# hyllios/CGAT

Hardware: AMD Instinct MI355X
Metric: edges/sec through one CGAT attention layer (fwd+bwd), 1M-edge batch (higher is better)
Workload: dtype f32 storage / f16x3c (24-bit operands: exact h + l + t split, 3 fp16 + 3 six-bit matrix passes where built, six bf16 passes elsewhere; fp32 accumulate); 1 GPU; one GATConvNodes layer (H_Net update) fwd+bwd, 4167 crystals x 20 atoms x 12 nbrs per rank: N=83340, E=1000080, C=Ce=128, H=3, scalar attention; edges_per_rank=1000080, parallelism=dp1 (graphs sharded, gradient all-reduce)

## Files before the change

cgat_amd/csrc/edgebwd.hip:

```cpp
#include <string.h>
#include "../../include/cgat_hip.h"
#include "common.h"
#include "kernels.h"
#include "mfma_bf16.h"

__device__ __forceinline__ float rc_d(unsigned m, int bit) {
  const unsigned s = (unsigned)((int)(m << (31 - bit)) >> 31);
  return __uint_as_float((s & 0x3F800000u) | (~s & 0x3C23D70Au));
}
__device__ __forceinline__ bf16x8 bits8_bf16(unsigned m) {
  uint4 w;
#define GE_BITPAIR(i_) ((((unsigned)((int)(m << (31 - 2 * (i_))) >> 31)) & 0x3F80u) |                     \
                        (((unsigned)((int)(m << (30 - 2 * (i_))) >> 31)) & 0x3F800000u))
  w.x = GE_BITPAIR(0); w.y = GE_BITPAIR(1); w.z = GE_BITPAIR(2); w.w = GE_BITPAIR(3);
#undef GE_BITPAIR
  return __builtin_bit_cast(bf16x8, w);
}
template <int PASSES, bool RC = false, bool BP = false>
__global__ __launch_bounds__(512, 2) void edge_ge_kernel(const float* __restrict__ gZ, long ldg, long gzb,
                                                         const uint4* __restrict__ Wq, int ncb,
                                                         float* __restrict__ out, long ldo,
                                                         const int* __restrict__ scatter, int E, int accumulate,
                                                         const float* __restrict__ bias,
                                                         const float* __restrict__ amax, const EdgeRC rc, HeadBatch hb) {
// ... 996 lines not shown
    {
      CGAT_PROF("edge_gw", stream);
      edge_gw_go(f, p, true, stream);
      CGAT_LAUNCH_CHECK();
    }
    hipLaunchKernelGGL(edge_gw_bit_reduce_kernel, dim3(p.W2 * 4), dim3(256), 0, stream, p.ws + f.slab, f.SM, p.ws + f.slabA, f.SA,
                       p.ws + f.csl, p.rc->wA, p.rc->H, p.rc->HHd, p.W2, f.te_only ? nullptr : p.out, p.ldo, p.te ? *p.te : GwTe{});
    CGAT_LAUNCH_CHECK();
    if (p.te) {
      hipLaunchKernelGGL(gw_te_add_kernel, dim3(cdiv(p.rc->HHd, 256)), dim3(256), 0, stream, p.te->part, p.rc->HHd, p.te->out);
      CGAT_LAUNCH_CHECK();
    }
    if (!f.te_only) return CGAT_OK;
  }
  {
    CGAT_PROF(p.perm ? "edge_gw" : "rows_gw", stream);
    edge_gw_go(f, p, false, stream);
    CGAT_LAUNCH_CHECK();
  }
  return splitk_reduce_launch(p.ws + f.slab, f.S, p.W2, 128, p.out, p.ldo, stream);
}

#define GJ_NODES 4
__global__ __launch_bounds__(256) void edge_gj_kernel(const EdgeRC rc, const int* __restrict__ src_rowptr,
                                                      const int* __restrict__ src_pos, int N, int W2,
                                                      float* __restrict__ Gj, long ldo, float* __restrict__ gjmax) {
  float gmax = 0.f;
  const int per_xcd = gridDim.x / 8;
  const int blk = (blockIdx.x & 7) * per_xcd + (blockIdx.x >> 3);
  const int n0 = blk * GJ_NODES, n1 = min(N, n0 + GJ_NODES);
  for (int q = threadIdx.x; 4 * q < W2; q += 256) {
    const int col = 4 * q;
    const bool isA = col < rc.HHd;
    const int cc = isA ? col : col - rc.HHd, h = cc / rc.Hd;
    const int word = col >> 5, bit = col & 31;
    const float* coef = (isA ? rc.ga : rc.alpha) + h;
    for (int n = n0; n < n1; ++n) {
      const int r0 = src_rowptr[n], r1 = src_rowptr[n + 1];
      float4 acc = make_float4(0.f, 0.f, 0.f, 0.f);
      for (int rb = r0; rb < r1; rb += 4) {
        long t[4];
        float k[4];
        unsigned m[4];
        float4 v[4];
#pragma unroll
        for (int u = 0; u < 4; ++u) t[u] = src_pos[rb + u < r1 ? rb + u : r1 - 1];
#pragma unroll
        for (int u = 0; u < 4; ++u) {
          k[u] = rb + u < r1 ? coef[t[u] * rc.H] : 0.f;
          m[u] = rc.mask[t[u] * rc.nw + word];
          v[u] = *reinterpret_cast<const float4*>(isA ? rc.wA + cc : rc.gS + (long)rc.dst[t[u]] * rc.HHd + cc);
        }
#pragma unroll
        for (int u = 0; u < 4; ++u) {
          const unsigned mb = m[u] >> bit;
          acc.x += (k[u] * v[u].x) * rc_d(mb, 0); acc.y += (k[u] * v[u].y) * rc_d(mb, 1);
          acc.z += (k[u] * v[u].z) * rc_d(mb, 2); acc.w += (k[u] * v[u].w) * rc_d(mb, 3);
        }
      }
      *reinterpret_cast<float4*>(Gj + (long)n * ldo + col) = acc;
      gmax = fmaxf(fmaxf(gmax, fmaxf(fabsf(acc.x), fabsf(acc.y))), fmaxf(fabsf(acc.z), fabsf(acc.w)));
    }
  }
  if (gjmax) block_absmax_commit(gmax, gjmax);
}
int edge_gj_launch(const EdgeRC& rc, const int* src_rowptr, const int* src_pos, int N, int W2, float* Gj, long ldo,
                   hipStream_t stream, float* gjmax) {
  if (N <= 0) return CGAT_OK;
  CGAT_CHECK_ARG(W2 % 4 == 0 && (ldo % 4) == 0 && (((uintptr_t)Gj) & 15) == 0,
                 "edge_gj: W2 = %d must be a multiple of 4 with a 16-byte aligned output", W2);
  CGAT_PROF("edge_gj", stream);
  hipLaunchKernelGGL(edge_gj_kernel, dim3(cdiv(cdiv(N, GJ_NODES), 8) * 8), dim3(256), 0, stream, rc, src_rowptr, src_pos,
                     N, W2, Gj, ldo, gjmax);
  CGAT_LAUNCH_CHECK();
  return CGAT_OK;
}

extern "C" int cgat_debug_edge_bwd_form(int32_t product, int32_t launch, int32_t rows, int32_t W2, int32_t H, int32_t Hd,
                                        int32_t rebuilt, int32_t maxima, int32_t perm, int32_t force_six, int32_t te,
                                        cgat_edge_bwd_form* out) {
  CGAT_CHECK_ARG(out && (product == 0 || product == 1) && launch >= 0 && launch <= (product == 0 ? 3 : 0) && rows >= 0 &&
                 W2 > 0 && W2 % 128 == 0 && H > 0 && Hd > 0, "debug_edge_bwd_form: bad arguments");
  alignas(16) static float present_f;
  static int present_i;
  const EdgeRC rc = edge_rc_shape_only(H, Hd, W2);
  memset(out, 0, sizeof(*out));
  if (product == 1) {
    const EdgeGwParams p = edge_gw_shape(rows, W2, rebuilt ? &rc : nullptr, maxima != 0, perm != 0, force_six != 0, te != 0);
    const EdgeGwForm f = edge_gw_form(p);
    CGAT_TRY(edge_gw_check(p, f));
    out->passes = f.passes; out->rc = f.rc; out->bitplane = f.bitplane; out->grid_x = f.grid_x;
    out->bit_shape = f.bit_shape; out->te_only = f.te_only; out->ranges = f.S; out->SA = f.SA; out->SM = f.SM;
    out->message_pairs = f.npm; out->bit_grid_x = f.bit_grid_x;
    out->ws_end = (int64_t)f.ws_end; out->ws_floats = (int64_t)edge_gw_ws_floats(rows, W2);
    return CGAT_OK;
  }
// ... 14 lines not shown
```

cgat_amd/csrc/kernels.h:

```cpp
#pragma once
#include "common.h"

#define CGAT_ACT_NONE 0
#define CGAT_ACT_TANH 1
#define CGAT_ACT_LEAKY 2
#define CGAT_ACT_RELU 3

struct GemmParams {
  int M, N, K;
  const float* A;
  long lda;
  int a_kmajor;
  const int* a_rgather;
  long a_block;
  const float* B;
  long ldb;
  int b_kmajor;
  const int* b_kgather;
  float* C;
  long ldc;
  const int* c_scatter;
  float alpha, beta;
  const float* bias;
  const float* add1;
// ... 248 lines not shown
  float* out;
  long ld_dact, ld_resid, ld_out;
  int act;
  int dact_type;
  int accumulate;
};
struct ChainDesc {
  ChainLayer layer[CHAIN_MAX];
  int n_layers, rows;
  const float* x;
  long ldx;
  const float* in_dact;
  long ld_in_dact;
  int in_dact_type;
  float* in_store;
  long ld_in_store;
};
int prepare_W_batch_launch(const WPrepBatch& b, float* dst, hipStream_t stream);
bool mlp_chain128_fast(const ChainDesc& d);
int mlp_chain128_launch(const ChainDesc& d, hipStream_t stream);
#define CHAIN_BATCH_MAX 4
int mlp_chain128_batch_launch(const ChainDesc* d, int n, hipStream_t stream);
int edge_seg_bwd_chunks(int N);
int edge_seg_bwd_launch(const float* Z, float* gZ, long gz_block, const float* alpha, const float* gS, const float* gs,
                        const int* rowptr, const float* wA_out, int N, int H, int Hd, float* tt, float* ga, float* Gi,
                        float* partialW, float* gzmax, unsigned* mask, float* gimax, bool vec, bool zb_6, bool zb,
                        bool rc_shape, bool have_scales, hipStream_t stream,
                        const int* bits_src = nullptr);
int attn_signs_launch(const float* Z, const int* perm, long E, int W2, uint8_t* mask, hipStream_t stream,
                      const unsigned* zbits = nullptr);
struct EdgeRC {
  const unsigned* mask;
  const float* ga;
  const float* alpha;
  const float* gS;
  const float* wA;
  const int* dst;
  int H, Hd, HHd, nw;
  const float* cs;
};
bool edge_mma_bf16();
static inline bool edge_rc_shape(int Ce, int H, int Hd) { return Ce == 128 && H > 0 && Hd > 0 && Hd % 128 == 0; }
struct GwTe {
  const float* We;
  long ldw;
  double* part;
  float* out;
};
struct EdgeGeParams {
  const float* gZ;
  long ldg, gzb;
// ... 67 lines not shown
  p.gZ = gZ; p.ldg = ldg; p.gzb = gzb; p.e = e; p.lde = lde; p.perm = perm; p.E = E; p.W2 = W2; p.ws = ws;
  p.out = out; p.ldo = ldo;
  return p;
}
struct EdgeGwForm {
  int passes;
  bool rc;
  bool bit_shape;
  bool bitplane;
  bool te_only;
  int S, grid_x;
  int SA, SM, npm;
  int bit_grid_x;
  size_t slab;
  size_t slabA, csl;
  size_t ws_end;
};
EdgeGwForm edge_gw_form(const EdgeGwParams& p);
bool edge_gw_bitplane_layer(int H, int Hd);
bool edge_gw_dims(int Ce, int W2, long ldg, long gzb);
size_t edge_gw_ws_floats(int E, int W2);
bool edge_gw_force_six(bool on);
int edge_gw_launch(const EdgeGwParams& p, hipStream_t stream);
int edge_gj_launch(const EdgeRC& rc, const int* src_rowptr, const int* src_pos, int N, int W2, float* Gj, long ldo,
                   hipStream_t stream, float* gjmax = nullptr);

bool rows_dw128_fast(const float* G, long ldg, const float* X1, long ldx1, const float* X2, long ldx2);
size_t rows_dw128_ws_bytes(int rows, int nx);
int rows_dw128_launch(const float* G, long ldg, const float* X1, long ldx1, float* out1, long ldo1, const float* X2,
                      long ldx2, float* out2, long ldo2, float* bsum, int rows, void* ws, size_t ws_bytes,
                      hipStream_t stream);
#define DW_BATCH_MAX 32
struct DwBatchItem {
  const float* G;
  const float* X;
  float* out;
  float* bsum;
};
struct DwBatchDesc {
  int n, rows, splits, rows_per_unit;
  long ldg, ldx, ldo;
  DwBatchItem it[DW_BATCH_MAX];
};
size_t rows_dw128_batch_ws_bytes(int n_items, int rows);
bool rows_dw128_batch_fast(const DwBatchDesc& d);
int rows_dw128_batch_launch(DwBatchDesc d, void* ws, size_t ws_bytes, hipStream_t stream);

int layernorm_tanh_fwd_launch(const float* u, float* y, int rows, int W, float eps, hipStream_t s);
// ... 59 lines not shown
```

cgat_amd/csrc/layers.hip:

```cpp
#include "layers.h"

struct AttnDims {
  int N, E, C, Ce, H, Hd, D, HHd, W2;
};
static AttnDims attn_dims(const cgat_plan* plan, const cgat_attn_params* p) {
  AttnDims d;
  d.N = plan->N; d.E = plan->E; d.C = p->C; d.Ce = p->Ce; d.H = p->H; d.Hd = p->Hd;
  d.D = 2 * p->C + p->Ce; d.HHd = p->H * p->Hd; d.W2 = 2 * d.HHd;
  return d;
}

struct AttnSaved {
  float *Z, *alpha, *S, *ssum;
};
static AttnSaved attn_saved(float* saved, const AttnDims& d) {
  AttnSaved s;
  s.Z = saved;
  s.alpha = s.Z + (size_t)d.E * d.W2;
  s.S = s.alpha + (size_t)d.E * d.H;
  s.ssum = s.S + (size_t)d.N * d.HHd;
  return s;
}

static int g_edge_storage = -1;
// ... 411 lines not shown
struct GzView {
  const float* ptr;
  long ld, block;
};
static EdgeRC edge_rc_make(const unsigned* mask, const float* ga, const float* alpha, const float* gS, const float* wA,
                           const int* dst, int H, int Hd) {
  EdgeRC rc = {};
  rc.mask = mask; rc.ga = ga; rc.alpha = alpha; rc.gS = gS; rc.wA = wA; rc.dst = dst;
  rc.H = H; rc.Hd = Hd; rc.HHd = H * Hd; rc.nw = 2 * H * Hd / 32;
  return rc;
}
struct EdgeTail {
  GzView gZ;
  float *Gi, *Gj;
  bool have_Gi;
  const float* Wcat;
  float *gWcat, *gbcat;
  float *Wq, *gw_ws;
  const float* scales;
  const EdgeRC* rc;
  bool node_scales;
  bool gw_force_six;
  GwTe te;
  const float *x, *e;
  float *g_x, *g_e;
};

enum NodeSide { NODE_KSPLIT, NODE_SMALL_ROWS, NODE_LAUNCHES, NODE_GEMM };
enum EdgeProduct { PRODUCT_KSPLIT, PRODUCT_LAUNCH, PRODUCT_GEMM };
struct TailRoute {
  NodeSide node;
  int Sx, Se;
  bool node_scales;
  EdgeProduct ge, gw;
};
static TailRoute tail_route(bool dry, const AttnDims& d, const EdgeTail& t) {
  TailRoute r = {};
  const bool maxima = t.scales && d.C == 128 && aligned16(t.x);
  r.node_scales = t.rc ? maxima
                       : maxima && t.node_scales && !dry && d.N > 0 && d.W2 % 128 == 0 && aligned16(t.Gi, t.Gj);
  r.Sx = (!r.node_scales && d.C == 128) ? edge_ge_ksplit_groups(d.N, d.W2, false) : 1;
  r.Se = (!t.scales && d.Ce == 128) ? edge_ge_ksplit_groups(d.E, d.W2, t.rc != nullptr) : 1;
  const bool node_fast = !dry && d.N > 0 && edge_ge_dims(d.C, d.W2, d.W2, 128, d.C) && edge_gw_dims(d.C, d.W2, d.W2, 128) &&
                         aligned16(t.Gi, t.g_x, t.Gj, t.x) && d.N <= d.E;
  r.node = !node_fast ? NODE_GEMM : r.Sx > 1 ? NODE_KSPLIT : d.N <= rowprog_max_rows() ? NODE_SMALL_ROWS : NODE_LAUNCHES;
  const bool ge_fast = !dry && edge_ge_dims(d.Ce, d.W2, t.gZ.ld, t.gZ.block, d.Ce) && aligned16(t.gZ.ptr, t.g_e);
  r.ge = !ge_fast ? PRODUCT_GEMM : r.Se > 1 ? PRODUCT_KSPLIT : PRODUCT_LAUNCH;
  r.gw = (!dry && edge_gw_dims(d.Ce, d.W2, t.gZ.ld, t.gZ.block) && aligned16(t.gZ.ptr)) ? PRODUCT_LAUNCH : PRODUCT_GEMM;
  return r;
}
static long tail_xblock(const AttnDims& d, const EdgeTail& t) {
  return (t.gZ.ld == d.W2) ? 0 : t.gZ.block;
}

static int tail_segment_sums(Ctx& c, const cgat_plan* plan, const AttnDims& d, const EdgeTail& t, const TailRoute& r) {
  const long xb = tail_xblock(d, t);
  float* ns = r.node_scales ? const_cast<float*>(t.scales) + 2 : nullptr;
  if (!t.have_Gi)
    RUN(seg_wsum_launch(t.gZ.ptr, d.W2, nullptr, nullptr, 0, 1, plan->dst_rowptr, d.N, d.W2, CGAT_ACT_NONE, t.Gi, d.W2, c.s,
                        xb));
  if (t.rc) {
    RUN(edge_gj_launch(*t.rc, plan->src_rowptr, plan->src_pos, d.N, d.W2, t.Gj, d.W2, c.s, ns ? ns + 1 : nullptr));
    return CGAT_OK;
  }
  RUN(seg_wsum_launch(t.gZ.ptr, d.W2, plan->src_pos, nullptr, 0, 1, plan->src_rowptr, d.N, d.W2, CGAT_ACT_NONE, t.Gj, d.W2,
                      c.s, xb));
  if (ns) {
    RUN(absmax_rows128_launch(t.Gi, 128, (int)((long)d.N * d.W2 / 128), ns, c.s));
    RUN(absmax_rows128_launch(t.Gj, 128, (int)((long)d.N * d.W2 / 128), ns + 1, c.s));
    RUN(absmax_rows128_launch(t.x, d.C, d.N, ns + 2, c.s));
  }
  return CGAT_OK;
}

static int tail_gx_gemm_pair(Ctx& c, const AttnDims& d, const EdgeTail& t) {
  GemmParams g = gemm_params(d.N, d.C, d.W2, t.Gi, d.W2, t.Wcat, d.D, t.g_x, d.C);
  g.b_kmajor = 1;
  CGAT_TRY(c.gemm(g));
  g = gemm_params(d.N, d.C, d.W2, t.Gj, d.W2, t.Wcat + d.C + d.Ce, d.D, t.g_x, d.C);
  g.b_kmajor = 1;
  g.beta = 1.f;
  return c.gemm(g);
}
static int tail_node_products(Ctx& c, const AttnDims& d, const EdgeTail& t, const TailRoute& r) {
  const float* ns = r.node_scales ? t.scales + 2 : nullptr;
// ... 75 lines not shown
    CGAT_CHECK_ARG(r.ge != PRODUCT_GEMM && r.gw != PRODUCT_GEMM && t.have_Gi,
                   "nodes_attention_backward: the rebuilt-gZ path needs the split per-edge kernels");
  CGAT_TRY(tail_edge_ge(c, plan, d, t, r));
  return tail_edge_gw(c, plan, d, t, r);
}

static int edge_first_layer_backward_tail(Ctx& c, const cgat_plan* plan, const AttnDims& d, const EdgeTail& t) {
  const TailRoute r = tail_route(c.dry, d, t);
  CGAT_TRY(tail_segment_sums(c, plan, d, t, r));
  CGAT_TRY(tail_node_products(c, d, t, r));
  return tail_edge_products(c, plan, d, t, r);
}

struct AttnBwd {
  AttnDims d;
  const cgat_plan* plan;
  const cgat_attn_params* p;
  const cgat_attn_grads* gr;
  const float *x, *e, *g_aggr;
  float *g_x, *g_e;
  float *Wcat, *gWcat, *gbcat, *gS, *gs, *gas, *tt, *ga, *gZ, *partial, *Gi, *Gj, *Wq, *gw_ws;
  float* scales;
  int chunks;
  long gzb, gz_ld;
  AttnSaved sv;
  EdgeRC rc;
  AttnBwdRoute r;
};
static AttnBwd attn_bwd_carve(Ctx& c, const cgat_plan* plan, const cgat_attn_params* p, const float* x, const float* e,
                              const float* saved, const float* g_aggr, float* g_x, float* g_e, const cgat_attn_grads* gr) {
  AttnBwd b = {};
  const AttnDims d = b.d = attn_dims(plan, p);
  b.plan = plan; b.p = p; b.gr = gr; b.x = x; b.e = e; b.g_aggr = g_aggr; b.g_x = g_x; b.g_e = g_e;
  b.chunks = edge_seg_bwd_chunks(d.N);
  if (!c.dry) b.sv = attn_saved(const_cast<float*>(saved), d);
  b.Wcat = c.take<float>((size_t)d.W2 * d.D);
  b.r = attn_bwd_route(c.dry, d, p, x, e, saved, b.sv.S, b.Wcat);
  b.gWcat = c.take<float>((size_t)d.W2 * d.D);
  b.gbcat = c.take<float>((size_t)d.W2);
  b.gS = c.take<float>((size_t)d.N * d.HHd);
  b.gs = c.take<float>((size_t)d.N * d.H);
  b.gas = mode_split() ? c.take<float>((size_t)d.N * d.C) : nullptr;
  b.tt = c.take<float>((size_t)d.E * d.H);
  b.ga = c.take<float>((size_t)d.E * d.H);
  b.gZ = c.take<float>(b.r.rc ? (size_t)d.E * (d.W2 / 32) : (size_t)d.E * d.W2);
  b.partial = c.take<float>((size_t)b.chunks * d.HHd);
  b.Gi = c.take<float>((size_t)d.N * d.W2);
  b.Gj = c.take<float>((size_t)d.N * d.W2);
  b.Wq = c.take<float>(edge_z_wq_floats(d.W2));
  b.gw_ws = c.take<float>(edge_gw_ws_floats(d.E, d.W2));
  b.scales = c.take<float>(64);
  c.seal();
  b.gzb = (d.W2 % 128 == 0) ? (long)d.E * 128 : 0;
  b.gz_ld = b.gzb ? 128 : d.W2;
  if (b.r.rc && !c.dry)
    b.rc = edge_rc_make(reinterpret_cast<const unsigned*>(b.gZ), b.ga, b.sv.alpha, b.gS, p->A_out_w, plan->dst_sorted, d.H, d.Hd);
  return b;
}

static int attn_bwd_out_layer(Ctx& c, const AttnBwd& b) {
  const AttnDims& d = b.d;
  const cgat_attn_params* p = b.p;
  const float invH = 1.f / d.H;
  if (attn_bwd_out_shape(d)) {
    c.need(rows_dw128_batch_ws_bytes(d.H * (d.Hd / 128), d.N));
    c.need(linear128_ws_bytes(d.Hd));
    c.need((size_t)d.H * linear128_heads_image_floats(d.Hd) * sizeof(float));
  }
  if (b.r.out_fast) {
    RUN(scale_launch(b.g_aggr, invH, b.gas, (long)d.N * d.C, c.s));
    if (b.r.out_heads_one) {
      Linear128Params l = linear128_params(b.gas, d.C, p->M_out_w, 1, d.Hd, b.gS, d.HHd, d.N, d.Hd);
      l.heads = d.H; l.s_w = (long)d.C * d.Hd; l.s_out = d.Hd;
      CGAT_TRY(linear128_heads_launch(l, c.scratch, c.s));
    } else {
      for (int h = 0; h < d.H; ++h) {
        GemmParams g = gemm_params(d.N, d.Hd, d.C, b.gas, d.C, p->M_out_w + (size_t)h * d.C * d.Hd, d.Hd,
                                   b.gS + (size_t)h * d.Hd, d.HHd);
        g.b_kmajor = 1;
// ... 24 lines not shown
    }
  }
  GemmParams g = gemm_params(d.N, d.H, d.C, b.g_aggr, d.C, p->M_out_b, d.C, b.gs, d.H);
  g.alpha = invH;
  CGAT_TRY(c.gemm(g));
  g = gemm_params(d.H, d.C, d.N, b.sv.ssum, d.H, b.g_aggr, d.C, b.gr->M_out_b, d.C);
  g.a_kmajor = 1; g.b_kmajor = 1;
  g.alpha = invH;
  return c.gemm(g, true);
}

static int attn_bwd_segments(Ctx& c, const AttnBwd& b) {
  const AttnDims& d = b.d;
  const AttnBwdRoute& r = b.r;
  if (!c.dry && d.N > 0) {
    if (edge_bf16_storage() && !r.z_bf16) {
      cgat_set_error("nodes_attention_backward: edge storage \"bf16\" is set but this layer has no bf16 form");
      return CGAT_ERR_UNSUPPORTED;
    }
    CGAT_CHECK_ARG(!r.z_bits || (r.rc && r.vec), "nodes_attention_backward: the bit form of the saved buffer without its route");
    CGAT_CHECK_ARG(!r.z_bits || ((size_t)d.E * d.H * sizeof(float) >= (size_t)4 * d.HHd * sizeof(double) &&
                                 (((uintptr_t)b.tt) & 7) == 0),
                   "nodes_attention_backward: the bit form needs %d doubles of scratch in tt", 4 * d.HHd);
    if (r.rc)
      CGAT_CHECK_ARG(r.vec && aligned16(b.e),
                     "nodes_attention_backward: saved, edge_attr and MH_A.fc_out.weight must be 16-byte aligned at these widths");
    unsigned* mask = r.rc ? reinterpret_cast<unsigned*>(b.gZ) : nullptr;
    float* gzmax = r.have_scales ? b.scales : nullptr;
    float* gimax = (r.have_scales && r.rc) ? b.scales + 2 : nullptr;
    CGAT_TRY(edge_seg_bwd_launch(b.sv.Z, b.gZ, b.gzb, b.sv.alpha, b.gS, b.gs, b.plan->dst_rowptr, b.p->A_out_w, d.N, d.H, d.Hd,
                                 b.tt, b.ga, b.Gi, b.partial, gzmax, mask, gimax, r.vec, r.z_bf16_six, r.z_bf16, r.rc,
                                 r.have_scales, c.s, r.z_bits ? b.plan->src_sorted : nullptr));
  }
  if (r.have_scales) RUN(absmax_rows128_launch(b.e, d.Ce, d.E, b.scales + 1, c.s));
  if (r.have_scales && r.rc && d.C == 128 && aligned16(b.x)) RUN(absmax_rows128_launch(b.x, d.C, d.N, b.scales + 4, c.s));
  CGAT_TRY(c.colsum(b.ga, d.H, d.E, d.H, b.gr->A_out_b, 1.f));
  return c.colsum(b.partial, d.HHd, d.N > 0 ? b.chunks : 0, d.HHd, b.gr->A_out_w, 1.f);
}

static EdgeTail attn_bwd_tail(const AttnBwd& b) {
  EdgeTail t = {};
  t.gZ = {b.r.rc ? nullptr : b.gZ, b.gz_ld, b.gzb};
  t.Gi = b.Gi; t.Gj = b.Gj; t.have_Gi = true;
  t.Wcat = b.Wcat; t.gWcat = b.gWcat; t.gbcat = b.gbcat;
  t.Wq = b.Wq; t.gw_ws = b.gw_ws;
  t.scales = b.r.have_scales ? b.scales : nullptr;
  t.rc = b.r.rc ? &b.rc : nullptr;
  t.x = b.x; t.e = b.e; t.g_x = b.g_x; t.g_e = b.g_e;
  if (b.r.z_bits && b.gr) t.te = {b.Wcat + b.d.C, b.d.D, reinterpret_cast<double*>(b.tt), b.gr->A_out_w};
  return t;
}

static int attn_bwd_scatter_grads(Ctx& c, const AttnBwd& b) {
  const AttnDims& d = b.d;
  Copy2DJobs j;
  j.n = 4;
  j.job[0] = {b.gWcat, d.D, b.gr->A_in_w, d.D, d.HHd, d.D};
  j.job[1] = {b.gWcat + (size_t)d.HHd * d.D, d.D, b.gr->M_in_w, d.D, d.HHd, d.D};
  j.job[2] = {b.gbcat, d.HHd, b.gr->A_in_b, d.HHd, 1, d.HHd};
  j.job[3] = {b.gbcat + d.HHd, d.HHd, b.gr->M_in_b, d.HHd, 1, d.HHd};
  RUN(copy2d_multi_launch(j, c.s));
  return CGAT_OK;
}

static int attn_backward_impl(Ctx& c, const cgat_plan* plan, const cgat_attn_params* p, const float* x, const float* e,
                              const float* saved, const float* g_aggr, float* g_x, float* g_e,
                              const cgat_attn_grads* gr) {
  const AttnBwd b = attn_bwd_carve(c, plan, p, x, e, saved, g_aggr, g_x, g_e, gr);
  CGAT_TRY(stack_in_weights(c, p, b.d, b.Wcat, nullptr));
  CGAT_TRY(attn_bwd_out_layer(c, b));
  CGAT_TRY(attn_bwd_segments(c, b));
  CGAT_TRY(edge_first_layer_backward_tail(c, plan, b.d, attn_bwd_tail(b)));
// ... 657 lines not shown
```

cgat_amd/csrc/segbwd.hip:

```cpp
#include "common.h"
#include "kernels.h"
#include "mfma_bf16.h"

#define SEGB_NODES 8
#define SEGB_LONG 256
__device__ __forceinline__ float wave_sum_l(float v) {
#pragma unroll
  for (int o = 32; o > 0; o >>= 1) v += __shfl_xor(v, o, 64);
  return v;
}
template <bool VEC, bool ZB = false>
__global__ __launch_bounds__(256) void edge_seg_bwd_kernel(const float* __restrict__ Z, float* __restrict__ gZ,
                                                           long gz_block, const float* __restrict__ alpha,
                                                           const float* __restrict__ gS, const float* __restrict__ gs,
                                                           const int* __restrict__ rowptr,
                                                           const float* __restrict__ wA_out, int N, int H, int Hd,
                                                           float* __restrict__ tt, float* __restrict__ ga,
                                                           float* __restrict__ Gi, float* __restrict__ partialW,
                                                           float* __restrict__ gzmax, unsigned* __restrict__ mask,
                                                           float* __restrict__ gimax) {
  extern __shared__ float pw[];
  float gm = 0.f, gim_max = 0.f;
  const int HHd = H * Hd, W2 = 2 * HHd;
  const int tid = threadIdx.x, lane = tid & 63, wave = tid >> 6;
// ... 361 lines not shown
            w |= (unsigned)__builtin_amdgcn_mov_dpp((int)w, 0xB1, 0xF, 0xF, true);
            w |= (unsigned)__builtin_amdgcn_mov_dpp((int)w, 0x4E, 0xF, 0xF, true);
            w |= (unsigned)__builtin_amdgcn_mov_dpp((int)w, 0x141, 0xF, 0xF, true);
            if ((lane & 7) == 0) mask[(long)t * (W2 >> 5) + (col >> 5)] = w;
            gm = fmaxf(fmaxf(gm, fmaxf(fabsf(g.x), fabsf(g.y))), fmaxf(fabsf(g.z), fabsf(g.w)));
            gi.x += g.x; gi.y += g.y; gi.z += g.z; gi.w += g.w;
          }
        }
      }
      *reinterpret_cast<float4*>(Gi + (long)n * W2 + col) = gi;
      gim_max = fmaxf(fmaxf(gim_max, fmaxf(fabsf(gi.x), fabsf(gi.y))), fmaxf(fabsf(gi.z), fabsf(gi.w)));
      pw[col] += ps.x; pw[col + 1] += ps.y; pw[col + 2] += ps.z; pw[col + 3] += ps.w;
    }
  }
  __syncthreads();
  for (int c = tid; c < HHd; c += 256) partialW[(long)blockIdx.x * HHd + c] = pw[c];
  if (gzmax) block_absmax_commit(gm, gzmax);
  if (gimax) {
    __syncthreads();
    block_absmax_commit(gim_max, gimax);
  }
}

__global__ __launch_bounds__(256, 8) void seg_bwd_attb_kernel(const float* __restrict__ saved, const float* __restrict__ ga,
                                                              const int* __restrict__ rowptr, const int* __restrict__ srcs,
                                                              const float* __restrict__ wA_out, int N, int H,
                                                              float* __restrict__ Gi, float* __restrict__ partialW,
                                                              unsigned* __restrict__ mask) {
  constexpr int Hd = 256;
  extern __shared__ float pw[];
  const int HHd = H * Hd, W2 = 2 * HHd;
  const int tid = threadIdx.x, lane = tid & 63;
  const float* PiA = saved;
  const float* PjA = saved + (long)N * W2;
  const unsigned* zb = reinterpret_cast<const unsigned*>(saved + 2l * N * W2);
  for (int c = tid; c < HHd; c += 256) pw[c] = 0.f;
  __syncthreads();
  const int n0 = blockIdx.x * SEGB_NODES, n1 = min(N, n0 + SEGB_NODES);
  for (int n = n0; n < n1; ++n) {
    const int r0 = __builtin_amdgcn_readfirstlane(rowptr[n]), r1 = __builtin_amdgcn_readfirstlane(rowptr[n + 1]);
    if (r1 == r0) {
      for (int c = tid; c < W2; c += 256) Gi[(long)n * W2 + c] = 0.f;
      continue;
    }
    for (int c4 = tid; c4 < HHd / 4; c4 += 256) {
      const int col = 4 * c4;
      const int h = col / Hd;
      const int bit = col & 31;
      const unsigned* zw = zb + (col >> 5) * 32;
      const unsigned woff = (unsigned)(col >> 5) * 4u;
      const float4 wv = *reinterpret_cast<const float4*>(wA_out + col);
      const float4 pi = *reinterpret_cast<const float4*>(PiA + (long)n * W2 + col);
      float4 gi = make_float4(0.f, 0.f, 0.f, 0.f), ps = gi;
      for (int tb = r0; tb < r1; tb += 4) {
        unsigned m[4];
        float cf[4];
        int sn[4];
        float4 pj[4];
#pragma unroll
        for (int u = 0; u < 4; ++u) {
          const int t = tb + u < r1 ? tb + u : r1 - 1;
          m[u] = zw[(long)(t >> 5) * W2 + (t & 31)];
          cf[u] = ga[(long)t * H + h];
          sn[u] = srcs[t];
        }
#pragma unroll
        for (int u = 0; u < 4; ++u)
          pj[u] = *reinterpret_cast<const float4*>(reinterpret_cast<const char*>(PjA) +
                                                   ((unsigned)sn[u] * (unsigned)W2 + (unsigned)col) * 4u);
#pragma unroll
        for (int u = 0; u < 4; ++u) {
          const int t = tb + u;
          if (t < r1) {
            const unsigned mb = m[u] >> bit;
            const float4 d = make_float4((mb & 1u) ? 1.f : 0.01f, (mb & 2u) ? 1.f : 0.01f, (mb & 4u) ? 1.f : 0.01f,
                                         (mb & 8u) ? 1.f : 0.01f);
            const float gav = cf[u];
            const float4 g = make_float4(gav * wv.x * d.x, gav * wv.y * d.y, gav * wv.z * d.z, gav * wv.w * d.w);
            ps.x += (gav * d.x) * (pi.x + pj[u].x); ps.y += (gav * d.y) * (pi.y + pj[u].y);
            ps.z += (gav * d.z) * (pi.z + pj[u].z); ps.w += (gav * d.w) * (pi.w + pj[u].w);
            if ((lane & 7) == 0) {
              unsigned wo = woff;
              asm volatile("" : "+v"(wo));
              *reinterpret_cast<unsigned*>(reinterpret_cast<char*>(mask + (long)t * (W2 >> 5)) + wo) = m[u];
            }
            gi.x += g.x; gi.y += g.y; gi.z += g.z; gi.w += g.w;
          }
        }
      }
      *reinterpret_cast<float4*>(Gi + (long)n * W2 + col) = gi;
      pw[col] += ps.x; pw[col + 1] += ps.y; pw[col + 2] += ps.z; pw[col + 3] += ps.w;
    }
  }
  __syncthreads();
  for (int c = tid; c < HHd; c += 256) partialW[(long)blockIdx.x * HHd + c] = pw[c];
}

__global__ void attn_signs_kernel(const float* __restrict__ Z, const int* __restrict__ perm, long E, int W2,
                                  uint8_t* __restrict__ mask, const unsigned* __restrict__ zbits) {
  const long i = (long)blockIdx.x * blockDim.x + threadIdx.x;
  if (i >= E * W2) return;
  const long t = i / W2;
  const int c = (int)(i - t * W2);
  if (zbits && c < W2 / 2) mask[(long)perm[t] * W2 + c] = (zbits[(t >> 5) * W2 + (c >> 5) * 32 + (t & 31)] >> (c & 31)) & 1u;
  else mask[(long)perm[t] * W2 + c] = Z[i] > 0.f ? 1 : 0;
}
int attn_signs_launch(const float* Z, const int* perm, long E, int W2, uint8_t* mask, hipStream_t stream,
                      const unsigned* zbits) {
  const long n = E * W2;
  if (n == 0) return CGAT_OK;
  hipLaunchKernelGGL(attn_signs_kernel, dim3((unsigned)cdiv(n, 256)), dim3(256), 0, stream, Z, perm, E, W2, mask, zbits);
  CGAT_LAUNCH_CHECK();
  return CGAT_OK;
}

int edge_seg_bwd_chunks(int N) { return cdiv(N > 0 ? N : 1, SEGB_NODES); }

int seg_bwd_soft_launch(const float* alpha, const float* tt, const int* rowptr, int N, int H, float* ga, hipStream_t stream) {
  CGAT_CHECK_ARG(H >= 1 && H <= 16, "seg_bwd_soft: more than 16 heads");
  if (N <= 0) return CGAT_OK;
  CGAT_PROF("edge_idx_bwd_soft", stream);
  hipLaunchKernelGGL(seg_bwd_soft_kernel, dim3(edge_seg_bwd_chunks(N)), dim3(256), 0, stream, alpha, tt, rowptr, N, H, ga);
  CGAT_LAUNCH_CHECK();
  return CGAT_OK;
}

template <bool ZB>
static int seg_bwd_three_launch(const float* Z, const float* alpha, const float* gS, const float* gs, const int* rowptr,
                                const float* wA_out, int N, int H, float* tt, float* ga, float* Gi, float* partialW,
                                float* gzmax, unsigned* mask, float* gimax, hipStream_t stream,
                                const int* srcs = nullptr) {
  const int chunks = edge_seg_bwd_chunks(N);
  hipLaunchKernelGGL(seg_bwd_msg_kernel<ZB>, dim3((unsigned)cdiv((long)N * H, 4)), dim3(256), 0, stream, Z, alpha, gS, gs, rowptr,
                     N, H, tt, Gi, gzmax, mask, gimax);
  CGAT_LAUNCH_CHECK();
  hipLaunchKernelGGL(seg_bwd_soft_kernel, dim3(chunks), dim3(256), 0, stream, alpha, tt, rowptr, N, H, ga);
  CGAT_LAUNCH_CHECK();
  if (srcs)
    hipLaunchKernelGGL(seg_bwd_attb_kernel, dim3(chunks), dim3(256), (size_t)H * 256 * sizeof(float), stream, Z, ga, rowptr,
                       srcs, wA_out, N, H, Gi, partialW, mask);
  else
  hipLaunchKernelGGL(seg_bwd_att_kernel<ZB>, dim3(chunks), dim3(256), (size_t)H * 256 * sizeof(float), stream, Z, ga, rowptr,
                     wA_out, N, H, Gi, partialW, gzmax, mask, gimax);
  CGAT_LAUNCH_CHECK();
  return CGAT_OK;
}

int edge_seg_bwd_launch(const float* Z, float* gZ, long gz_block, const float* alpha, const float* gS, const float* gs,
                        const int* rowptr, const float* wA_out, int N, int H, int Hd, float* tt, float* ga, float* Gi,
                        float* partialW, float* gzmax, unsigned* mask, float* gimax, bool vec, bool zb_6, bool zb,
                        bool rc_shape, bool have_scales, hipStream_t stream, const int* bits_src) {
  CGAT_CHECK_ARG(H <= 16, "nodes_attention_backward: more than 16 heads");
  CGAT_CHECK_ARG(!bits_src || (vec && mask && Hd == 256 && !zb && !zb_6 && !have_scales),
                 "nodes_attention_backward: the bit form of the saved buffer is the three-kernel fp32 route's");
  CGAT_PROF("edge_seg_bwd", stream);
  if (have_scales) CGAT_TRY(fill_launch(gzmax, 0.f, 8, stream));
  const int chunks = edge_seg_bwd_chunks(N);
  const size_t shm = (size_t)H * Hd * sizeof(float);
  if (zb_6) {
    CGAT_CHECK_ARG(vec && mask && Hd == 256, "nodes_attention_backward: the bf16 edge storage needs the vector form");
    return seg_bwd_three_launch<true>(Z, alpha, gS, gs, rowptr, wA_out, N, H, tt, ga, Gi, partialW, gzmax, mask, gimax, stream);
  }
  if (zb) {
    CGAT_CHECK_ARG(rc_shape && have_scales, "nodes_attention_backward: the bf16 edge storage needs the vector form");
    hipLaunchKernelGGL((edge_seg_bwd_kernel<true, true>), dim3(chunks), dim3(256), shm, stream, Z, gZ, gz_block, alpha, gS,
                       gs, rowptr, wA_out, N, H, Hd, tt, ga, Gi, partialW, gzmax, mask, gimax);
  } else if (vec && mask && Hd == 256) {
    return seg_bwd_three_launch<false>(Z, alpha, gS, gs, rowptr, wA_out, N, H, tt, ga, Gi, partialW, gzmax, mask, gimax, stream,
                                       bits_src);
  } else if (vec)
    hipLaunchKernelGGL(edge_seg_bwd_kernel<true>, dim3(chunks), dim3(256), shm, stream, Z, gZ, gz_block, alpha, gS, gs,
                       rowptr, wA_out, N, H, Hd, tt, ga, Gi, partialW, gzmax, mask, gimax);
  else
    hipLaunchKernelGGL(edge_seg_bwd_kernel<false>, dim3(chunks), dim3(256), shm, stream, Z, gZ, gz_block, alpha, gS, gs,
                       rowptr, wA_out, N, H, Hd, tt, ga, Gi, partialW, (float*)nullptr, (unsigned*)nullptr, (float*)nullptr);
  CGAT_LAUNCH_CHECK();
  return CGAT_OK;
}
```

Before: 36.14 million edges/s.

## Split attention weight-gradient sum into Pi and Pj halves, drop source gather

The bit-form attention backward kernel used to gather the source node's Pj projection for every edge to form the weight-gradient partials. The gradient term is now split algebraically. The destination half (sum of ga*d times Pi) stays in a rewritten one-wave-per-node-head attb kernel that walks the bit mask in 16-edge groups with shuffles. The source half (sum of ga*d times Pj) is accumulated inside the edge_gj kernel, which already walks edges grouped by source, and its partial rows are written to a shared workspace that a single colsum reduces. This removes the per-edge random Pj gathers and the shared-memory block reduction, at the cost of extra registers and FMAs in edge_gj, a different rounding order, and a new workspace-size constraint.

```diff
diff --git a/cgat_amd/csrc/edgebwd.hip b/cgat_amd/csrc/edgebwd.hip
--- a/cgat_amd/csrc/edgebwd.hip
+++ b/cgat_amd/csrc/edgebwd.hip
@@ -1042,9 +1042,12 @@
 }
 
 #define GJ_NODES 4
-__global__ __launch_bounds__(256) void edge_gj_kernel(const EdgeRC rc, const int* __restrict__ src_rowptr,
+int edge_gj_uj_rows(int N) { return cdiv(cdiv(N > 0 ? N : 1, GJ_NODES), 8) * 8; }
+template <bool UJ>
+__global__ __launch_bounds__(256, UJ ? 8 : 1) void edge_gj_kernel(const EdgeRC rc, const int* __restrict__ src_rowptr,
                                                       const int* __restrict__ src_pos, int N, int W2,
-                                                      float* __restrict__ Gj, long ldo, float* __restrict__ gjmax) {
+                                                      float* __restrict__ Gj, long ldo, float* __restrict__ gjmax,
+                                                      const GjUj uj) {
   float gmax = 0.f;
   const int per_xcd = gridDim.x / 8;
   const int blk = (blockIdx.x & 7) * per_xcd + (blockIdx.x >> 3);
@@ -1055,6 +1058,41 @@
     const int cc = isA ? col : col - rc.HHd, h = cc / rc.Hd;
     const int word = col >> 5, bit = col & 31;
     const float* coef = (isA ? rc.ga : rc.alpha) + h;
+    if (UJ && isA) {
+      const float4 wv = *reinterpret_cast<const float4*>(rc.wA + cc);
+      float4 pw = make_float4(0.f, 0.f, 0.f, 0.f);
+      for (int n = n0; n < n1; ++n) {
+        const int r0 = src_rowptr[n], r1 = src_rowptr[n + 1];
+        float4 acc = make_float4(0.f, 0.f, 0.f, 0.f), us = acc, pj = acc;
+        for (int rb = r0; rb < r1; rb += 4) {
+          long t[4];
+          float k[4];
+          unsigned m[4];
+#pragma unroll
+          for (int u = 0; u < 4; ++u) t[u] = src_pos[rb + u < r1 ? rb + u : r1 - 1];
+#pragma unroll
+          for (int u = 0; u < 4; ++u) {
+            k[u] = rb + u < r1 ? coef[t[u] * rc.H] : 0.f;
+            m[u] = rc.mask[t[u] * rc.nw + word];
+          }
+          if (rb == r0) pj = *reinterpret_cast<const float4*>(uj.PjA + (long)n * uj.ld + col);
+#pragma unroll
+          for (int u = 0; u < 4; ++u) {
+            const unsigned mb = m[u] >> bit;
+            acc.x += (k[u] * wv.x) * rc_d(mb, 0); acc.y += (k[u] * wv.y) * rc_d(mb, 1);
+            acc.z += (k[u] * wv.z) * rc_d(mb, 2); acc.w += (k[u] * wv.w) * rc_d(mb, 3);
+            us.x = __fmaf_rn(k[u], rc_d(mb, 0), us.x); us.y = __fmaf_rn(k[u], rc_d(mb, 1), us.y);
+            us.z = __fmaf_rn(k[u], rc_d(mb, 2), us.z); us.w = __fmaf_rn(k[u], rc_d(mb, 3), us.w);
+          }
+        }
+        *reinterpret_cast<float4*>(Gj + (long)n * ldo + col) = acc;
+        gmax = fmaxf(fmaxf(gmax, fmaxf(fabsf(acc.x), fabsf(acc.y))), fmaxf(fabsf(acc.z), fabsf(acc.w)));
+        pw.x = __fmaf_rn(us.x, pj.x, pw.x); pw.y = __fmaf_rn(us.y, pj.y, pw.y);
+        pw.z = __fmaf_rn(us.z, pj.z, pw.z); pw.w = __fmaf_rn(us.w, pj.w, pw.w);
+      }
+      *reinterpret_cast<float4*>(uj.part + (long)blk * rc.HHd + col) = pw;
+      continue;
+    }
     for (int n = n0; n < n1; ++n) {
       const int r0 = src_rowptr[n], r1 = src_rowptr[n + 1];
       float4 acc = make_float4(0.f, 0.f, 0.f, 0.f);
@@ -1085,13 +1123,20 @@
   if (gjmax) block_absmax_commit(gmax, gjmax);
 }
 int edge_gj_launch(const EdgeRC& rc, const int* src_rowptr, const int* src_pos, int N, int W2, float* Gj, long ldo,
-                   hipStream_t stream, float* gjmax) {
+                   hipStream_t stream, float* gjmax, const GjUj* uj) {
   if (N <= 0) return CGAT_OK;
   CGAT_CHECK_ARG(W2 % 4 == 0 && (ldo % 4) == 0 && (((uintptr_t)Gj) & 15) == 0,
                  "edge_gj: W2 = %d must be a multiple of 4 with a 16-byte aligned output", W2);
+  CGAT_CHECK_ARG(!uj || (uj->PjA && uj->part && uj->ld % 4 == 0 && rc.HHd % 4 == 0 &&
+                         ((((uintptr_t)uj->PjA) | ((uintptr_t)uj->part)) & 15) == 0),
+                 "edge_gj: the half projection and the partial rows must be 16-byte aligned");
   CGAT_PROF("edge_gj", stream);
-  hipLaunchKernelGGL(edge_gj_kernel, dim3(cdiv(cdiv(N, GJ_NODES), 8) * 8), dim3(256), 0, stream, rc, src_rowptr, src_pos,
-                     N, W2, Gj, ldo, gjmax);
+  const dim3 grid(edge_gj_uj_rows(N));
+  if (uj)
+    hipLaunchKernelGGL(edge_gj_kernel<true>, grid, dim3(256), 0, stream, rc, src_rowptr, src_pos, N, W2, Gj, ldo, gjmax, *uj);
+  else
+    hipLaunchKernelGGL(edge_gj_kernel<false>, grid, dim3(256), 0, stream, rc, src_rowptr, src_pos, N, W2, Gj, ldo, gjmax,
+                       GjUj{});
   CGAT_LAUNCH_CHECK();
   return CGAT_OK;
 }
diff --git a/cgat_amd/csrc/kernels.h b/cgat_amd/csrc/kernels.h
--- a/cgat_amd/csrc/kernels.h
+++ b/cgat_amd/csrc/kernels.h
@@ -294,11 +294,11 @@
 #define CHAIN_BATCH_MAX 4
 int mlp_chain128_batch_launch(const ChainDesc* d, int n, hipStream_t stream);
 int edge_seg_bwd_chunks(int N);
+int seg_bwd_attb_rows(int N, int H);
 int edge_seg_bwd_launch(const float* Z, float* gZ, long gz_block, const float* alpha, const float* gS, const float* gs,
                         const int* rowptr, const float* wA_out, int N, int H, int Hd, float* tt, float* ga, float* Gi,
                         float* partialW, float* gzmax, unsigned* mask, float* gimax, bool vec, bool zb_6, bool zb,
-                        bool rc_shape, bool have_scales, hipStream_t stream,
-                        const int* bits_src = nullptr);
+                        bool rc_shape, bool have_scales, hipStream_t stream, bool bits = false);
 int attn_signs_launch(const float* Z, const int* perm, long E, int W2, uint8_t* mask, hipStream_t stream,
                       const unsigned* zbits = nullptr);
 struct EdgeRC {
@@ -412,8 +412,15 @@
 size_t edge_gw_ws_floats(int E, int W2);
 bool edge_gw_force_six(bool on);
 int edge_gw_launch(const EdgeGwParams& p, hipStream_t stream);
+struct GjUj {
+  const float* PjA;
+  long ld;
+  float* part;
+};
+int edge_gj_uj_rows(int N);
 int edge_gj_launch(const EdgeRC& rc, const int* src_rowptr, const int* src_pos, int N, int W2, float* Gj, long ldo,
-                   hipStream_t stream, float* gjmax = nullptr);
+                   hipStream_t stream, float* gjmax = nullptr,
+                   const GjUj* uj = nullptr);
 
 bool rows_dw128_fast(const float* G, long ldg, const float* X1, long ldx1, const float* X2, long ldx2);
 size_t rows_dw128_ws_bytes(int rows, int nx);
diff --git a/cgat_amd/csrc/layers.hip b/cgat_amd/csrc/layers.hip
--- a/cgat_amd/csrc/layers.hip
+++ b/cgat_amd/csrc/layers.hip
@@ -457,6 +457,9 @@
   bool node_scales;
   bool gw_force_six;
   GwTe te;
+  GjUj uj;
+  const float* wa_part;
+  int wa_rows;
   const float *x, *e;
   float *g_x, *g_e;
 };
@@ -495,7 +498,9 @@
     RUN(seg_wsum_launch(t.gZ.ptr, d.W2, nullptr, nullptr, 0, 1, plan->dst_rowptr, d.N, d.W2, CGAT_ACT_NONE, t.Gi, d.W2, c.s,
                         xb));
   if (t.rc) {
-    RUN(edge_gj_launch(*t.rc, plan->src_rowptr, plan->src_pos, d.N, d.W2, t.Gj, d.W2, c.s, ns ? ns + 1 : nullptr));
+    RUN(edge_gj_launch(*t.rc, plan->src_rowptr, plan->src_pos, d.N, d.W2, t.Gj, d.W2, c.s, ns ? ns + 1 : nullptr,
+                       t.uj.part ? &t.uj : nullptr));
+    if (t.uj.part) CGAT_TRY(c.colsum(t.wa_part, d.HHd, t.wa_rows, d.HHd, t.te.out, 1.f));
     return CGAT_OK;
   }
   RUN(seg_wsum_launch(t.gZ.ptr, d.W2, plan->src_pos, nullptr, 0, 1, plan->src_rowptr, d.N, d.W2, CGAT_ACT_NONE, t.Gj, d.W2,
@@ -617,6 +622,7 @@
   float *Wcat, *gWcat, *gbcat, *gS, *gs, *gas, *tt, *ga, *gZ, *partial, *Gi, *Gj, *Wq, *gw_ws;
   float* scales;
   int chunks;
+  int uj_rows;
   long gzb, gz_ld;
   AttnSaved sv;
   EdgeRC rc;
@@ -650,6 +656,12 @@
   b.gz_ld = b.gzb ? 128 : d.W2;
   if (b.r.rc && !c.dry)
     b.rc = edge_rc_make(reinterpret_cast<const unsigned*>(b.gZ), b.ga, b.sv.alpha, b.gS, p->A_out_w, plan->dst_sorted, d.H, d.Hd);
+  if (b.r.z_bits) {
+    b.chunks = seg_bwd_attb_rows(d.N, d.H);
+    b.uj_rows = edge_gj_uj_rows(d.N);
+    b.partial = b.gw_ws;
+  }
+  if (attn_bit_form_dims(d)) c.need(colsum_ws_bytes(seg_bwd_attb_rows(d.N, d.H) + edge_gj_uj_rows(d.N), d.HHd));
   return b;
 }
 
@@ -720,6 +732,8 @@
     CGAT_CHECK_ARG(!r.z_bits || ((size_t)d.E * d.H * sizeof(float) >= (size_t)4 * d.HHd * sizeof(double) &&
                                  (((uintptr_t)b.tt) & 7) == 0),
                    "nodes_attention_backward: the bit form needs %d doubles of scratch in tt", 4 * d.HHd);
+    CGAT_CHECK_ARG(!r.z_bits || (size_t)(b.chunks + b.uj_rows) * d.HHd <= edge_gw_ws_floats(d.E, d.W2),
+                   "nodes_attention_backward: the partial rows of the bit form do not fit grad W_e's workspace");
     if (r.rc)
       CGAT_CHECK_ARG(r.vec && aligned16(b.e),
                      "nodes_attention_backward: saved, edge_attr and MH_A.fc_out.weight must be 16-byte aligned at these widths");
@@ -728,11 +742,12 @@
     float* gimax = (r.have_scales && r.rc) ? b.scales + 2 : nullptr;
     CGAT_TRY(edge_seg_bwd_launch(b.sv.Z, b.gZ, b.gzb, b.sv.alpha, b.gS, b.gs, b.plan->dst_rowptr, b.p->A_out_w, d.N, d.H, d.Hd,
                                  b.tt, b.ga, b.Gi, b.partial, gzmax, mask, gimax, r.vec, r.z_bf16_six, r.z_bf16, r.rc,
-                                 r.have_scales, c.s, r.z_bits ? b.plan->src_sorted : nullptr));
+                                 r.have_scales, c.s, r.z_bits));
   }
   if (r.have_scales) RUN(absmax_rows128_launch(b.e, d.Ce, d.E, b.scales + 1, c.s));
   if (r.have_scales && r.rc && d.C == 128 && aligned16(b.x)) RUN(absmax_rows128_launch(b.x, d.C, d.N, b.scales + 4, c.s));
   CGAT_TRY(c.colsum(b.ga, d.H, d.E, d.H, b.gr->A_out_b, 1.f));
+  if (r.z_bits) return CGAT_OK;
   return c.colsum(b.partial, d.HHd, d.N > 0 ? b.chunks : 0, d.HHd, b.gr->A_out_w, 1.f);
 }
 
@@ -745,7 +760,11 @@
   t.scales = b.r.have_scales ? b.scales : nullptr;
   t.rc = b.r.rc ? &b.rc : nullptr;
   t.x = b.x; t.e = b.e; t.g_x = b.g_x; t.g_e = b.g_e;
-  if (b.r.z_bits && b.gr) t.te = {b.Wcat + b.d.C, b.d.D, reinterpret_cast<double*>(b.tt), b.gr->A_out_w};
+  if (b.r.z_bits && b.gr) {
+    t.te = {b.Wcat + b.d.C, b.d.D, reinterpret_cast<double*>(b.tt), b.gr->A_out_w};
+    t.uj = {b.sv.Z + (size_t)b.d.N * b.d.W2, b.d.W2, b.partial + (size_t)b.chunks * b.d.HHd};
+    t.wa_part = b.partial; t.wa_rows = b.chunks + b.uj_rows;
+  }
   return t;
 }
 
diff --git a/cgat_amd/csrc/segbwd.hip b/cgat_amd/csrc/segbwd.hip
--- a/cgat_amd/csrc/segbwd.hip
+++ b/cgat_amd/csrc/segbwd.hip
@@ -407,78 +407,79 @@
   }
 }
 
+template <class GA>
+__device__ __forceinline__ void segb_att_walk(const unsigned* __restrict__ zbh, unsigned* __restrict__ maskh, int W2,
+                                              int r0, int r1, int lane, const float4 wv, float4& gi, float4& ui,
+                                              GA ga_of) {
+  const int lr = lane >> 3, lw = lane & 7, bit = 4 * lw;
+  for (int tb = r0; tb < r1; tb += 16) {
+    unsigned mw[2];
+#pragma unroll
+    for (int c = 0; c < 2; ++c) {
+      const int t = tb + 8 * c + lr;
+      mw[c] = 0u;
+      if (t < r1) {
+        mw[c] = zbh[(long)(t >> 5) * W2 + lw * 32 + (t & 31)];
+        maskh[(long)t * (W2 >> 5) + lw] = mw[c];
+      }
+    }
+    const float gl = (lane < 16 && tb + lane < r1) ? ga_of(tb + lane) : 0.f;
+#pragma unroll
+    for (int c = 0; c < 2; ++c) {
+#pragma unroll
+      for (int r = 0; r < 8; ++r) {
+        if (tb + 8 * c + r < r1) {
+          const unsigned mb = (unsigned)__shfl((int)mw[c], 8 * r + lr) >> bit;
+          const float4 d = make_float4((mb & 1u) ? 1.f : 0.01f, (mb & 2u) ? 1.f : 0.01f, (mb & 4u) ? 1.f : 0.01f,
+                                       (mb & 8u) ? 1.f : 0.01f);
+          const float gav = __int_as_float(__builtin_amdgcn_readlane(__float_as_int(gl), 8 * c + r));
+          const float4 g = make_float4(gav * wv.x * d.x, gav * wv.y * d.y, gav * wv.z * d.z, gav * wv.w * d.w);
+          ui.x = __fmaf_rn(gav, d.x, ui.x); ui.y = __fmaf_rn(gav, d.y, ui.y);
+          ui.z = __fmaf_rn(gav, d.z, ui.z); ui.w = __fmaf_rn(gav, d.w, ui.w);
+          gi.x += g.x; gi.y += g.y; gi.z += g.z; gi.w += g.w;
+        }
+      }
+    }
+  }
+}
+
+#define SEGB_ATT_WGS 2048
+int seg_bwd_attb_rows(int N, int H) {
+  const int k = cdiv(N > 0 ? N : 1, 4), cap = SEGB_ATT_WGS / (H > 0 ? H : 1);
+  return 4 * (k < cap ? k : (cap > 0 ? cap : 1));
+}
 __global__ __launch_bounds__(256, 8) void seg_bwd_attb_kernel(const float* __restrict__ saved, const float* __restrict__ ga,
-                                                              const int* __restrict__ rowptr, const int* __restrict__ srcs,
+                                                              const int* __restrict__ rowptr,
                                                               const float* __restrict__ wA_out, int N, int H,
                                                               float* __restrict__ Gi, float* __restrict__ partialW,
                                                               unsigned* __restrict__ mask) {
   constexpr int Hd = 256;
-  extern __shared__ float pw[];
   const int HHd = H * Hd, W2 = 2 * HHd;
-  const int tid = threadIdx.x, lane = tid & 63;
+  const int lane = threadIdx.x & 63;
+  const int slot = __builtin_amdgcn_readfirstlane((int)blockIdx.x * 4 + (int)(threadIdx.x >> 6));
+  const int rows = (int)gridDim.x * 4 / H;
+  const int h = slot % H, p = slot / H;
+  const int col = h * Hd + 4 * lane;
   const float* PiA = saved;
-  const float* PjA = saved + (long)N * W2;
-  const unsigned* zb = reinterpret_cast<const unsigned*>(saved + 2l * N * W2);
-  for (int c = tid; c < HHd; c += 256) pw[c] = 0.f;
-  __syncthreads();
-  const int n0 = blockIdx.x * SEGB_NODES, n1 = min(N, n0 + SEGB_NODES);
-  for (int n = n0; n < n1; ++n) {
+  const unsigned* zbh = reinterpret_cast<const unsigned*>(saved + 2l * N * W2) + h * (Hd / 32) * 32;
+  unsigned* maskh = mask + h * (Hd / 32);
+  const float4 wv = *reinterpret_cast<const float4*>(wA_out + col);
+  float4 ps = make_float4(0.f, 0.f, 0.f, 0.f);
+  for (int n = p; n < N; n += rows) {
     const int r0 = __builtin_amdgcn_readfirstlane(rowptr[n]), r1 = __builtin_amdgcn_readfirstlane(rowptr[n + 1]);
     if (r1 == r0) {
-      for (int c = tid; c < W2; c += 256) Gi[(long)n * W2 + c] = 0.f;
+      *reinterpret_cast<float4*>(Gi + (long)n * W2 + col) = make_float4(0.f, 0.f, 0.f, 0.f);
+      *reinterpret_cast<float4*>(Gi + (long)n * W2 + HHd + col) = make_float4(0.f, 0.f, 0.f, 0.f);
       continue;
     }
-    for (int c4 = tid; c4 < HHd / 4; c4 += 256) {
-      const int col = 4 * c4;
-      const int h = col / Hd;
-      const int bit = col & 31;
-      const unsigned* zw = zb + (col >> 5) * 32;
-      const unsigned woff = (unsigned)(col >> 5) * 4u;
-      const float4 wv = *reinterpret_cast<const float4*>(wA_out + col);
-      const float4 pi = *reinterpret_cast<const float4*>(PiA + (long)n * W2 + col);
-      float4 gi = make_float4(0.f, 0.f, 0.f, 0.f), ps = gi;
-      for (int tb = r0; tb < r1; tb += 4) {
-        unsigned m[4];
-        float cf[4];
-        int sn[4];
-        float4 pj[4];
-#pragma unroll
-        for (int u = 0; u < 4; ++u) {
-          const int t = tb + u < r1 ? tb + u : r1 - 1;
-          m[u] = zw[(long)(t >> 5) * W2 + (t & 31)];
-          cf[u] = ga[(long)t * H + h];
-          sn[u] = srcs[t];
-        }
-#pragma unroll
-        for (int u = 0; u < 4; ++u)
-          pj[u] = *reinterpret_cast<const float4*>(reinterpret_cast<const char*>(PjA) +
-                                                   ((unsigned)sn[u] * (unsigned)W2 + (unsigned)col) * 4u);
-#pragma unroll
-        for (int u = 0; u < 4; ++u) {
-          const int t = tb + u;
-          if (t < r1) {
-            const unsigned mb = m[u] >> bit;
-            const float4 d = make_float4((mb & 1u) ? 1.f : 0.01f, (mb & 2u) ? 1.f : 0.01f, (mb & 4u) ? 1.f : 0.01f,
-                                         (mb & 8u) ? 1.f : 0.01f);
-            const float gav = cf[u];
-            const float4 g = make_float4(gav * wv.x * d.x, gav * wv.y * d.y, gav * wv.z * d.z, gav * wv.w * d.w);
-            ps.x += (gav * d.x) * (pi.x + pj[u].x); ps.y += (gav * d.y) * (pi.y + pj[u].y);
-            ps.z += (gav * d.z) * (pi.z + pj[u].z); ps.w += (gav * d.w) * (pi.w + pj[u].w);
-            if ((lane & 7) == 0) {
-              unsigned wo = woff;
-              asm volatile("" : "+v"(wo));
-              *reinterpret_cast<unsigned*>(reinterpret_cast<char*>(mask + (long)t * (W2 >> 5)) + wo) = m[u];
-            }
-            gi.x += g.x; gi.y += g.y; gi.z += g.z; gi.w += g.w;
-          }
-        }
-      }
-      *reinterpret_cast<float4*>(Gi + (long)n * W2 + col) = gi;
-      pw[col] += ps.x; pw[col + 1] += ps.y; pw[col + 2] += ps.z; pw[col + 3] += ps.w;
-    }
-  }
-  __syncthreads();
-  for (int c = tid; c < HHd; c += 256) partialW[(long)blockIdx.x * HHd + c] = pw[c];
+    const float4 pi = *reinterpret_cast<const float4*>(PiA + (long)n * W2 + col);
+    float4 gi = make_float4(0.f, 0.f, 0.f, 0.f), ui = gi;
+    segb_att_walk(zbh, maskh, W2, r0, r1, lane, wv, gi, ui, [&](int t) { return ga[(long)t * H + h]; });
+    *reinterpret_cast<float4*>(Gi + (long)n * W2 + col) = gi;
+    ps.x = __fmaf_rn(ui.x, pi.x, ps.x); ps.y = __fmaf_rn(ui.y, pi.y, ps.y);
+    ps.z = __fmaf_rn(ui.z, pi.z, ps.z); ps.w = __fmaf_rn(ui.w, pi.w, ps.w);
+  }
+  *reinterpret_cast<float4*>(partialW + (long)p * HHd + col) = ps;
 }
 
 __global__ void attn_signs_kernel(const float* __restrict__ Z, const int* __restrict__ perm, long E, int W2,
@@ -514,16 +515,16 @@
 static int seg_bwd_three_launch(const float* Z, const float* alpha, const float* gS, const float* gs, const int* rowptr,
                                 const float* wA_out, int N, int H, float* tt, float* ga, float* Gi, float* partialW,
                                 float* gzmax, unsigned* mask, float* gimax, hipStream_t stream,
-                                const int* srcs = nullptr) {
+                                bool bits = false) {
   const int chunks = edge_seg_bwd_chunks(N);
   hipLaunchKernelGGL(seg_bwd_msg_kernel<ZB>, dim3((unsigned)cdiv((long)N * H, 4)), dim3(256), 0, stream, Z, alpha, gS, gs, rowptr,
                      N, H, tt, Gi, gzmax, mask, gimax);
   CGAT_LAUNCH_CHECK();
   hipLaunchKernelGGL(seg_bwd_soft_kernel, dim3(chunks), dim3(256), 0, stream, alpha, tt, rowptr, N, H, ga);
   CGAT_LAUNCH_CHECK();
-  if (srcs)
-    hipLaunchKernelGGL(seg_bwd_attb_kernel, dim3(chunks), dim3(256), (size_t)H * 256 * sizeof(float), stream, Z, ga, rowptr,
-                       srcs, wA_out, N, H, Gi, partialW, mask);
+  if (bits)
+    hipLaunchKernelGGL(seg_bwd_attb_kernel, dim3((unsigned)(seg_bwd_attb_rows(N, H) / 4 * H)), dim3(256), 0, stream, Z, ga,
+                       rowptr, wA_out, N, H, Gi, partialW, mask);
   else
   hipLaunchKernelGGL(seg_bwd_att_kernel<ZB>, dim3(chunks), dim3(256), (size_t)H * 256 * sizeof(float), stream, Z, ga, rowptr,
                      wA_out, N, H, Gi, partialW, gzmax, mask, gimax);
@@ -534,9 +535,9 @@
 int edge_seg_bwd_launch(const float* Z, float* gZ, long gz_block, const float* alpha, const float* gS, const float* gs,
                         const int* rowptr, const float* wA_out, int N, int H, int Hd, float* tt, float* ga, float* Gi,
                         float* partialW, float* gzmax, unsigned* mask, float* gimax, bool vec, bool zb_6, bool zb,
-                        bool rc_shape, bool have_scales, hipStream_t stream, const int* bits_src) {
+                        bool rc_shape, bool have_scales, hipStream_t stream, bool bits) {
   CGAT_CHECK_ARG(H <= 16, "nodes_attention_backward: more than 16 heads");
-  CGAT_CHECK_ARG(!bits_src || (vec && mask && Hd == 256 && !zb && !zb_6 && !have_scales),
+  CGAT_CHECK_ARG(!bits || (vec && mask && Hd == 256 && !zb && !zb_6 && !have_scales),
                  "nodes_attention_backward: the bit form of the saved buffer is the three-kernel fp32 route's");
   CGAT_PROF("edge_seg_bwd", stream);
   if (have_scales) CGAT_TRY(fill_launch(gzmax, 0.f, 8, stream));
@@ -552,7 +553,7 @@
                        gs, rowptr, wA_out, N, H, Hd, tt, ga, Gi, partialW, gzmax, mask, gimax);
   } else if (vec && mask && Hd == 256) {
     return seg_bwd_three_launch<false>(Z, alpha, gS, gs, rowptr, wA_out, N, H, tt, ga, Gi, partialW, gzmax, mask, gimax, stream,
-                                       bits_src);
+                                       bits);
   } else if (vec)
     hipLaunchKernelGGL(edge_seg_bwd_kernel<true>, dim3(chunks), dim3(256), shm, stream, Z, gZ, gz_block, alpha, gS, gs,
                        rowptr, wA_out, N, H, Hd, tt, ga, Gi, partialW, gzmax, mask, gimax);
```

Result: no change. 36.34 million edges/s, median of 6 (+0.5%).
